# Tamerkobba/Parallel-CNN

Hardware: AMD Instinct MI355X
Metric: training images/sec (whole node) (higher is better)
Workload: dtype bf16; 1 GPU; model=LeNet-5 28x28x1 (conv6x5x5 -> trainable-pool4x4 -> fc216x10), global_batch=64, per_gpu_batch=64, input=28x28x1, parallelism=dp1, dist_backend=none, pool=trainable, loss=residual, backend=hip, hipgraph=False, overlap_comm=False

## Files before the change

csrc/bindings.cpp:

```cpp

#include <torch/extension.h>

#include <cmath>

#include "lenet_dims.h"
#include "pcnn_launch.h"

namespace pcnn {
void cpu_forward(at::Tensor x, at::Tensor params, at::Tensor a1, at::Tensor a2,
                 at::Tensor y, int64_t pool_mode, int64_t loss_mode);
double cpu_backward(at::Tensor x, at::Tensor params, at::Tensor a1,
                    at::Tensor a2, at::Tensor y, at::Tensor labels,
                    at::Tensor dz, at::Tensor dz2, at::Tensor dz1,
                    at::Tensor grads, int64_t pool_mode, int64_t loss_mode);
void cpu_update(at::Tensor params, at::Tensor grads, double dt, double scale);
void cpu_update_momentum(at::Tensor params, at::Tensor grads, at::Tensor vel,
                         double dt, double scale, double mu, double wd,
                         bool nesterov);
void cpu_update_adam(at::Tensor params, at::Tensor grads, at::Tensor m,
                     at::Tensor sq, double dt, double scale, double beta1,
                     double beta2, double eps, double wd, int64_t t);
}

namespace {
// ... 200 lines not shown
void hip_wgrad_update_adam(at::Tensor x, at::Tensor a1, at::Tensor a2,
                           at::Tensor dz, at::Tensor dz2, at::Tensor dz1,
                           at::Tensor grads, at::Tensor params, at::Tensor m,
                           at::Tensor sq, double dt, double scale,
                           double beta1, double beta2, double eps, double wd,
                           int64_t t, at::Tensor ticket, int64_t B,
                           int64_t chunk_imgs, int64_t roles,
                           int64_t stream) {
  wgrad_update_impl(
      x, a1, a2, dz, dz2, dz1, grads, params,
      adam_opt(m, sq, params, dt, scale, beta1, beta2, eps, wd, t), ticket, B,
      chunk_imgs, roles, stream, "wgrad_update_adam");
}

float* gslab_ptr(const at::Tensor& gslab, int64_t B) {
  TORCH_CHECK(gslab.is_cuda() && gslab.scalar_type() == at::kFloat &&
                  gslab.is_contiguous() &&
                  gslab.numel() >= B * pcnn::GSLAB_LD,
              "gslab must be a contiguous device fp32 [>=B, ",
              pcnn::GSLAB_LD, "] tensor");
  return gslab.data_ptr<float>();
}

int inblock_variant(int64_t variant) {
  TORCH_CHECK(variant >= -1 && variant <= 1,
              "variant must be -1 (default), 0 (cell) or 1 (pair)");
  return (int)variant;
}

void hip_fwdbwd_inblock(at::Tensor x, at::Tensor params, at::Tensor a2,
                        at::Tensor y, at::Tensor dz, at::Tensor labels,
                        at::Tensor loss_accum, at::Tensor gslab, int64_t B,
                        int64_t stream, int64_t pool_mode,
                        int64_t loss_mode, int64_t variant) {
  TORCH_CHECK(x.is_cuda() && params.is_cuda(), "expected device tensors");
  TORCH_CHECK(labels.scalar_type() == at::kInt, "labels must be int32");
  TORCH_CHECK(B >= 1 && x.numel() >= B * pcnn::IN_PIX &&
                  a2.numel() >= B * pcnn::S1_OUT &&
                  a2.scalar_type() == x.scalar_type() &&
                  y.numel() >= B * pcnn::FC_OUT &&
                  dz.numel() >= B * pcnn::FC_OUT && labels.numel() >= B,
              "buffers too small for B");
  check_hip(pcnn_launch_fwdbwd_inblock(
                x.data_ptr(), params.data_ptr<float>(), a2.data_ptr(),
                y.data_ptr<float>(), dz.data_ptr<float>(),
                labels.data_ptr<int>(),
                loss_accum.numel() ? loss_accum.data_ptr<float>() : nullptr,
                gslab_ptr(gslab, B), (int)B, act_flag(x), (int)pool_mode,
                (int)loss_mode, inblock_variant(variant), (void*)stream),
            "fwdbwd_inblock");
}

void step_inblock_impl(const at::Tensor& x, const at::Tensor& params,
                       const at::Tensor& a1, const at::Tensor& a2,
                       const at::Tensor& y, const at::Tensor& dz,
                       const at::Tensor& dz2, const at::Tensor& dz1,
                       const at::Tensor& labels, const at::Tensor& loss_accum,
                       const at::Tensor& grads, const at::Tensor& ticket,
                       const at::Tensor& gslab, const pcnn_opt& opt,
                       int64_t B, int64_t chunk_imgs, int64_t stream,
                       int64_t pool_mode, int64_t loss_mode, int64_t variant,
                       const char* what) {
  TORCH_CHECK(x.is_cuda() && params.is_cuda(), "expected device tensors");
  TORCH_CHECK(labels.scalar_type() == at::kInt, "labels must be int32");
  TORCH_CHECK(dz1.scalar_type() == x.scalar_type() &&
                  a2.scalar_type() == x.scalar_type(),
              "a2/dz1 must match the activation dtype");
  TORCH_CHECK(params.numel() == pcnn::N_PARAMS &&
                  grads.numel() == pcnn::N_PARAMS,
              "params/grads must be the flat device buckets");
  TORCH_CHECK(B >= 1 && x.numel() >= B * pcnn::IN_PIX &&
                  a2.numel() >= B * pcnn::S1_OUT &&
                  y.numel() >= B * pcnn::FC_OUT &&
                  dz.numel() >= B * pcnn::FC_OUT && labels.numel() >= B,
              "buffers too small for B");
  TORCH_CHECK(B <= pcnn_inblock_max_batch() ||
                  (a1.numel() >= B * pcnn::C1_OUT &&
                   dz1.numel() >= B * pcnn::C1_OUT &&
                   dz2.numel() >= B * pcnn::S1_OUT),
              "a1/dz1/dz2 too small for the large-batch path");
  check_hip(pcnn_launch_step_inblock(
                x.data_ptr(), params.data_ptr<float>(), a1.data_ptr(),
                a2.data_ptr(), y.data_ptr<float>(), dz.data_ptr<float>(),
                dz2.data_ptr<float>(), dz1.data_ptr(), labels.data_ptr<int>(),
                loss_accum.data_ptr<float>(), grads.data_ptr<float>(),
                ticket_ptr(ticket), gslab_ptr(gslab, B), &opt, (int)B,
                act_flag(x), (int)pool_mode, (int)loss_mode, (int)chunk_imgs,
                inblock_variant(variant), (void*)stream),
            what);
}

void hip_step_inblock(at::Tensor x, at::Tensor params, at::Tensor a1,
                      at::Tensor a2, at::Tensor y, at::Tensor dz,
                      at::Tensor dz2, at::Tensor dz1, at::Tensor labels,
                      at::Tensor loss_accum, at::Tensor grads,
                      at::Tensor ticket, at::Tensor gslab, double step,
                      int64_t B, int64_t chunk_imgs, int64_t stream,
                      int64_t pool_mode, int64_t loss_mode,
                      int64_t variant) {
  step_inblock_impl(x, params, a1, a2, y, dz, dz2, dz1, labels, loss_accum,
                    grads, ticket, gslab, plain_opt(step), B, chunk_imgs,
                    stream, pool_mode, loss_mode, variant, "step_inblock");
}

void hip_step_inblock_momentum(at::Tensor x, at::Tensor params,
                               at::Tensor vel, at::Tensor a1, at::Tensor a2,
                               at::Tensor y, at::Tensor dz, at::Tensor dz2,
                               at::Tensor dz1, at::Tensor labels,
                               at::Tensor loss_accum, at::Tensor grads,
                               at::Tensor ticket, at::Tensor gslab, double dt,
                               double scale, double mu, double wd,
                               bool nesterov, int64_t B, int64_t chunk_imgs,
                               int64_t stream, int64_t pool_mode,
                               int64_t loss_mode, int64_t variant) {
  step_inblock_impl(x, params, a1, a2, y, dz, dz2, dz1, labels, loss_accum,
                    grads, ticket, gslab,
                    momentum_opt(vel, params, dt, scale, mu, wd, nesterov), B,
                    chunk_imgs, stream, pool_mode, loss_mode, variant,
                    "step_inblock_momentum");
}

void hip_step_inblock_adam(at::Tensor x, at::Tensor params, at::Tensor m,
                           at::Tensor sq, at::Tensor a1, at::Tensor a2,
                           at::Tensor y, at::Tensor dz, at::Tensor dz2,
                           at::Tensor dz1, at::Tensor labels,
                           at::Tensor loss_accum, at::Tensor grads,
                           at::Tensor ticket, at::Tensor gslab, double dt,
                           double scale, double beta1, double beta2,
                           double eps, double wd, int64_t t, int64_t B,
                           int64_t chunk_imgs, int64_t stream,
                           int64_t pool_mode, int64_t loss_mode,
                           int64_t variant) {
  step_inblock_impl(
      x, params, a1, a2, y, dz, dz2, dz1, labels, loss_accum, grads, ticket,
      gslab, adam_opt(m, sq, params, dt, scale, beta1, beta2, eps, wd, t), B,
      chunk_imgs, stream, pool_mode, loss_mode, variant, "step_inblock_adam");
}

void reduce_update_impl(const at::Tensor& gslab, const at::Tensor& a2,
                        const at::Tensor& dz, const at::Tensor& params,
                        const pcnn_opt& opt, int64_t B, int64_t stream,
                        const char* what) {
  TORCH_CHECK(params.is_cuda() && params.numel() == pcnn::N_PARAMS,
              "params must be the flat device bucket");
  TORCH_CHECK(B >= 1 && a2.is_cuda() && a2.numel() >= B * pcnn::S1_OUT &&
                  dz.is_cuda() && dz.scalar_type() == at::kFloat &&
                  dz.numel() >= B * pcnn::FC_OUT,
              "buffers too small for B");
  check_hip(pcnn_launch_reduce_update(gslab_ptr(gslab, B), a2.data_ptr(),
                                      dz.data_ptr<float>(),
                                      params.data_ptr<float>(), &opt, (int)B,
                                      act_flag(a2), (void*)stream),
            what);
}

void hip_reduce_update_momentum(at::Tensor gslab, at::Tensor a2,
                                at::Tensor dz, at::Tensor params,
                                at::Tensor vel, double dt, double scale,
                                double mu, double wd, bool nesterov,
                                int64_t B, int64_t stream) {
  reduce_update_impl(gslab, a2, dz, params,
                     momentum_opt(vel, params, dt, scale, mu, wd, nesterov),
                     B, stream, "reduce_update_momentum");
}

void hip_reduce_update_adam(at::Tensor gslab, at::Tensor a2, at::Tensor dz,
                            at::Tensor params, at::Tensor m, at::Tensor sq,
                            double dt, double scale, double beta1,
                            double beta2, double eps, double wd, int64_t t,
                            int64_t B, int64_t stream) {
  reduce_update_impl(
      gslab, a2, dz, params,
      adam_opt(m, sq, params, dt, scale, beta1, beta2, eps, wd, t), B, stream,
      "reduce_update_adam");
}

void hip_train_steps(at::Tensor x_pool, at::Tensor labels_pool,
                     at::Tensor params, at::Tensor grads, at::Tensor a1,
                     at::Tensor a2, at::Tensor y, at::Tensor dz,
                     at::Tensor dz2, at::Tensor dz1, at::Tensor loss_accum,
                     int64_t B, int64_t steps, int64_t chunk_imgs,
                     double step_scale, int64_t stream, int64_t pool_mode,
                     int64_t loss_mode, int64_t wgrad_fuse,
                     int64_t step_mode, at::Tensor ticket,
                     at::Tensor gslab, at::Tensor vel, double dt,
                     double scale, double mu, double wd, bool nesterov,
                     int64_t variant, at::Tensor sq, double beta2, double eps,
                     int64_t t0) {
  const int var = inblock_variant(variant);
  const bool adam = sq.numel() != 0;
  TORCH_CHECK(!adam || t0 >= 0, "t0 is the number of updates applied so far");
  pcnn_opt opt =
      adam ? adam_opt(vel, sq, params, dt, scale, mu, beta2, eps, wd, t0 + 1)
      : vel.numel() ? momentum_opt(vel, params, dt, scale, mu, wd, nesterov)
                    : plain_opt(step_scale);
  TORCH_CHECK(step_mode == 3 || step_mode == 2 || step_mode == 4,
              "step_mode must be 3, 2 or 4");
  TORCH_CHECK(step_mode == 3 || !wgrad_fuse,
              "the two-launch steps exclude wgrad_fuse");
  int* tk = step_mode != 3 ? ticket_ptr(ticket) : nullptr;
  float* slab = step_mode == 4 ? gslab_ptr(gslab, B) : nullptr;
  const int wroles = wgrad_fuse ? 4 : (pool_mode == 1 ? 5 : 7);
  TORCH_CHECK(x_pool.is_cuda() && x_pool.dim() == 2, "x_pool [P*B, 784]");
  TORCH_CHECK(labels_pool.scalar_type() == at::kInt, "labels must be int32");
  const int64_t pool_rows = x_pool.size(0);
  TORCH_CHECK(pool_rows % B == 0, "pool rows must be a multiple of B");
  const int64_t P = pool_rows / B;
  const int f = act_flag(x_pool);
  const size_t esz = f ? 2 : 4;
  const char* xp = (const char*)x_pool.data_ptr();
  const int* lp = labels_pool.data_ptr<int>();
  float* pp = params.data_ptr<float>();
  float* gp = grads.data_ptr<float>();
  void* s = (void*)stream;
  for (int64_t st = 0; st < steps; ++st) {
    const int64_t i = st % P;
    const void* xb = xp + (size_t)i * B * pcnn::IN_PIX * esz;
    const int* lb = lp + i * B;
    if (adam && st > 0)
      opt = adam_opt(vel, sq, params, dt, scale, mu, beta2, eps, wd,
                     t0 + st + 1);
    if (step_mode == 4) {
      check_hip(pcnn_launch_step_inblock(
                    xb, pp, a1.data_ptr(), a2.data_ptr(), y.data_ptr<float>(),
                    dz.data_ptr<float>(), dz2.data_ptr<float>(),
                    dz1.data_ptr(), lb, loss_accum.data_ptr<float>(), gp, tk,
                    slab, &opt, (int)B, f, (int)pool_mode, (int)loss_mode,
                    (int)chunk_imgs, var, s),
                "train_steps/step_inblock");
      continue;
    }
    check_hip(pcnn_launch_fwdbwd(xb, pp, a1.data_ptr(), a2.data_ptr(),
                                 y.data_ptr<float>(), dz.data_ptr<float>(),
                                 dz2.data_ptr<float>(), dz1.data_ptr(), lb,
                                 loss_accum.data_ptr<float>(), nullptr,
                                 (int)B, f, 0, (int)pool_mode, (int)loss_mode,
                                 gp, (int)wgrad_fuse, s),
              "train_steps/fwdbwd");
    if (step_mode == 2) {
      check_hip(pcnn_launch_wgrad_update(
                    xb, a1.data_ptr(), a2.data_ptr(), dz.data_ptr<float>(),
                    dz2.data_ptr<float>(), dz1.data_ptr(), gp, pp, &opt, tk,
                    (int)B, f, (int)chunk_imgs, wroles, s),
                "train_steps/wgrad_update");
      continue;
    }
    check_hip(pcnn_launch_wgrad(xb, a1.data_ptr(), a2.data_ptr(),
                                dz.data_ptr<float>(), dz2.data_ptr<float>(),
                                dz1.data_ptr(), gp, (int)B, f,
                                (int)chunk_imgs, wroles, s),
              "train_steps/wgrad");
    check_hip(pcnn_launch_update(pp, gp, &opt, s), "train_steps/update");
  }
}

void deep_im2col(at::Tensor x, at::Tensor cols, int64_t B, int64_t H,
                 int64_t W, int64_t Cin, int64_t K, int64_t P, int64_t KcP,
                 int64_t stream) {
  check_hip(pcnn_deep_im2col(x.data_ptr(), cols.data_ptr(), (int)B, (int)H,
                             (int)W, (int)Cin, (int)K, (int)P, (int)KcP,
                             act_flag(x), (void*)stream),
            "deep_im2col");
}

void deep_gemm(at::Tensor A, at::Tensor Bsrc, at::Tensor bias, at::Tensor C,
               int64_t M, int64_t K, int64_t N, int64_t ldA, int64_t ldC,
               int64_t b_kxn, int64_t epilogue, int64_t stream,
               at::Tensor Bpre, at::Tensor imx, int64_t XH, int64_t XW,
               int64_t XC, int64_t XK, int64_t XP, at::Tensor epi,
               at::Tensor pw, at::Tensor pout, int64_t PK, at::Tensor c32) {
  check_hip(pcnn_deep_gemm(
                A.data_ptr(), Bsrc.data_ptr<float>(),
                Bpre.numel() ? Bpre.data_ptr() : nullptr,
                bias.numel() ? bias.data_ptr<float>() : nullptr,
                C.data_ptr(), M, (int)K, (int)N, (int)ldA, (int)ldC,
                (int)b_kxn, (int)epilogue,
                imx.numel() ? imx.data_ptr() : nullptr, (int)XH, (int)XW,
                (int)XC, (int)XK, (int)XP,
                epi.numel() ? epi.data_ptr() : nullptr,
                pw.numel() ? pw.data_ptr<float>() : nullptr,
                pout.numel() ? pout.data_ptr() : nullptr, (int)PK,
                c32.numel() ? c32.data_ptr<float>() : nullptr,
                (long long)c32.numel(), act_flag(A), (void*)stream),
            "deep_gemm");
}

void deep_cast_wt(at::Tensor W, at::Tensor out, at::Tensor outT, int64_t R,
                  int64_t C, int64_t stream) {
  check_hip(pcnn_deep_cast_wt(W.data_ptr<float>(), out.data_ptr(),
                              outT.data_ptr(), (int)R, (int)C,
                              (void*)stream),
            "deep_cast_wt");
}

struct CastDesc {
  int R[8], C[8], K[8], Cin[8];
  long long w_off[8], bf_off[8], bfT_off[8], rot_off[8], p8_off[8];
  pcnn_cast_desc d;

  CastDesc(const char* what, const std::vector<int64_t>& Rv,
           const std::vector<int64_t>& Cv, const std::vector<int64_t>& Kv,
           const std::vector<int64_t>& Cinv, const std::vector<int64_t>& w,
           const std::vector<int64_t>& bf, const std::vector<int64_t>& bfT,
           const std::vector<int64_t>& rot, const std::vector<int64_t>& p8) {
    const size_t n = Rv.size();
    TORCH_CHECK(n >= 1 && n <= 8, what, ": 1..8 stages");
// ... 237 lines not shown
  check_hip(pcnn_deep_fc_fwd(
                flat.data_ptr(), fw.data_ptr<float>(), fb.data_ptr<float>(),
                labels.data_ptr<int>(),
                y.numel() ? y.data_ptr<float>() : nullptr,
                dz.numel() ? dz.data_ptr<float>() : nullptr,
                loss_accum.numel() ? loss_accum.data_ptr<float>() : nullptr,
                correct_accum.numel() ? correct_accum.data_ptr<int>()
                                      : nullptr,
                (int)B, (int)FCIN, (int)NCLS, (int)mode,
                dflat.numel() ? dflat.data_ptr() : nullptr, act_flag(flat),
                (void*)stream),
            "deep_fc_fwd");
}

void deep_fc_bwd(at::Tensor dz, at::Tensor flat, at::Tensor fw,
                 at::Tensor dflat, int64_t B, int64_t FCIN, int64_t NCLS,
                 int64_t stream) {
  check_hip(pcnn_deep_fc_bwd(dz.data_ptr<float>(), flat.data_ptr(),
                             fw.data_ptr<float>(), dflat.data_ptr(), (int)B,
                             (int)FCIN, (int)NCLS, act_flag(flat),
                             (void*)stream),
            "deep_fc_bwd");
}

void deep_fc_wgrad(at::Tensor dz, at::Tensor flat, at::Tensor gfw,
                   at::Tensor gfb, int64_t B, int64_t FCIN, int64_t NCLS,
                   int64_t FS, int64_t stream) {
  check_hip(pcnn_deep_fc_wgrad(dz.data_ptr<float>(), flat.data_ptr(),
                               gfw.data_ptr<float>(), gfb.data_ptr<float>(),
                               (int)B, (int)FCIN, (int)NCLS, (int)FS,
                               act_flag(flat), (void*)stream),
            "deep_fc_wgrad");
}

void deep_update(at::Tensor params, at::Tensor grads, double step,
                 int64_t stream) {
  const pcnn_opt opt = plain_opt(step);
  check_hip(pcnn_deep_update(params.data_ptr<float>(),
                             grads.data_ptr<float>(), params.numel(), &opt,
                             (void*)stream),
            "deep_update");
}

void deep_update_momentum(at::Tensor params, at::Tensor grads,
                          at::Tensor vel, double dt, double scale, double mu,
                          double wd, bool nesterov, int64_t stream) {
  TORCH_CHECK(grads.numel() == params.numel(), "grads/params size mismatch");
  const pcnn_opt opt = momentum_opt(vel, params, dt, scale, mu, wd, nesterov);
  check_hip(pcnn_deep_update(params.data_ptr<float>(),
                             grads.data_ptr<float>(), params.numel(), &opt,
                             (void*)stream),
            "deep_update_momentum");
}

void deep_update_adam(at::Tensor params, at::Tensor grads, at::Tensor m,
                      at::Tensor sq, double dt, double scale, double beta1,
                      double beta2, double eps, double wd, int64_t t,
                      int64_t stream) {
  TORCH_CHECK(grads.numel() == params.numel(), "grads/params size mismatch");
  const pcnn_opt opt =
      adam_opt(m, sq, params, dt, scale, beta1, beta2, eps, wd, t);
  check_hip(pcnn_deep_update(params.data_ptr<float>(),
                             grads.data_ptr<float>(), params.numel(), &opt,
                             (void*)stream),
            "deep_update_adam");
}

void deep_mfma_selftest(at::Tensor A, at::Tensor Bm, at::Tensor D,
                        int64_t stream) {
  check_hip(pcnn_deep_mfma_selftest(A.data_ptr<float>(),
                                    Bm.data_ptr<float>(),
                                    D.data_ptr<float>(), (void*)stream),
            "deep_mfma_selftest");
}


}

PYBIND11_MODULE(TORCH_EXTENSION_NAME, m) {
  m.doc() = "parallel_cnn_amd native ops (CPU reference + gfx950 HIP kernels)";
  m.def("cpu_forward", &pcnn::cpu_forward, py::arg("x"), py::arg("params"),
        py::arg("a1"), py::arg("a2"), py::arg("y"), py::arg("pool_mode") = 0,
        py::arg("loss_mode") = 0);
  m.def("cpu_backward", &pcnn::cpu_backward, py::arg("x"), py::arg("params"),
        py::arg("a1"), py::arg("a2"), py::arg("y"), py::arg("labels"),
        py::arg("dz"), py::arg("dz2"), py::arg("dz1"), py::arg("grads"),
        py::arg("pool_mode") = 0, py::arg("loss_mode") = 0);
  m.def("cpu_update", &pcnn::cpu_update);
  m.def("cpu_update_momentum", &pcnn::cpu_update_momentum, py::arg("params"),
        py::arg("grads"), py::arg("vel"), py::arg("dt"), py::arg("scale"),
        py::arg("mu"), py::arg("wd"), py::arg("nesterov"));
  m.def("cpu_update_adam", &pcnn::cpu_update_adam, py::arg("params"),
        py::arg("grads"), py::arg("m"), py::arg("sq"), py::arg("dt"),
        py::arg("scale"), py::arg("beta1"), py::arg("beta2"), py::arg("eps"),
        py::arg("wd"), py::arg("t"));
  m.def("hip_fwdbwd", &hip_fwdbwd, py::arg("x"), py::arg("params"),
        py::arg("a1"), py::arg("a2"), py::arg("y"), py::arg("dz"),
        py::arg("dz2"), py::arg("dz1"), py::arg("labels"),
        py::arg("loss_accum"), py::arg("correct_accum"), py::arg("B"),
        py::arg("mode"), py::arg("stream"), py::arg("pool_mode") = 0,
        py::arg("loss_mode") = 0, py::arg("grads") = at::empty({0}),
        py::arg("wgrad_fuse") = 0);
  m.def("hip_wgrad", &hip_wgrad);
  m.def("hip_wgrad_roles", &hip_wgrad_roles);
  m.def("hip_update", &hip_update);
  m.def("hip_train_steps", &hip_train_steps, py::arg("x_pool"),
        py::arg("labels_pool"), py::arg("params"), py::arg("grads"),
        py::arg("a1"), py::arg("a2"), py::arg("y"), py::arg("dz"),
        py::arg("dz2"), py::arg("dz1"), py::arg("loss_accum"), py::arg("B"),
        py::arg("steps"), py::arg("chunk_imgs"), py::arg("step_scale"),
        py::arg("stream"), py::arg("pool_mode") = 0,
        py::arg("loss_mode") = 0, py::arg("wgrad_fuse") = 0,
        py::arg("step_mode") = 3, py::arg("ticket") = at::empty({0}),
        py::arg("gslab") = at::empty({0}), py::arg("vel") = at::empty({0}),
        py::arg("dt") = 0.0, py::arg("scale") = 1.0, py::arg("mu") = 0.0,
        py::arg("wd") = 0.0, py::arg("nesterov") = false,
        py::arg("variant") = -1, py::arg("sq") = at::empty({0}),
        py::arg("beta2") = 0.999, py::arg("eps") = 1e-8, py::arg("t0") = 0);
  m.def("hip_update_adam", &hip_update_adam, py::arg("params"),
        py::arg("grads"), py::arg("m"), py::arg("sq"), py::arg("dt"),
        py::arg("scale"), py::arg("beta1"), py::arg("beta2"), py::arg("eps"),
        py::arg("wd"), py::arg("t"), py::arg("stream"));
  m.def("hip_wgrad_update_adam", &hip_wgrad_update_adam, py::arg("x"),
        py::arg("a1"), py::arg("a2"), py::arg("dz"), py::arg("dz2"),
        py::arg("dz1"), py::arg("grads"), py::arg("params"), py::arg("m"),
        py::arg("sq"), py::arg("dt"), py::arg("scale"), py::arg("beta1"),
        py::arg("beta2"), py::arg("eps"), py::arg("wd"), py::arg("t"),
        py::arg("ticket"), py::arg("B"), py::arg("chunk_imgs"),
        py::arg("roles"), py::arg("stream"));
  m.def("hip_reduce_update_adam", &hip_reduce_update_adam, py::arg("gslab"),
        py::arg("a2"), py::arg("dz"), py::arg("params"), py::arg("m"),
        py::arg("sq"), py::arg("dt"), py::arg("scale"), py::arg("beta1"),
        py::arg("beta2"), py::arg("eps"), py::arg("wd"), py::arg("t"),
        py::arg("B"), py::arg("stream"));
  m.def("hip_step_inblock_adam", &hip_step_inblock_adam, py::arg("x"),
        py::arg("params"), py::arg("m"), py::arg("sq"), py::arg("a1"),
        py::arg("a2"), py::arg("y"), py::arg("dz"), py::arg("dz2"),
        py::arg("dz1"), py::arg("labels"), py::arg("loss_accum"),
        py::arg("grads"), py::arg("ticket"), py::arg("gslab"), py::arg("dt"),
        py::arg("scale"), py::arg("beta1"), py::arg("beta2"), py::arg("eps"),
        py::arg("wd"), py::arg("t"), py::arg("B"), py::arg("chunk_imgs"),
        py::arg("stream"), py::arg("pool_mode") = 0,
        py::arg("loss_mode") = 0, py::arg("variant") = -1);
  m.def("hip_update_momentum", &hip_update_momentum, py::arg("params"),
        py::arg("grads"), py::arg("vel"), py::arg("dt"), py::arg("scale"),
        py::arg("mu"), py::arg("wd"), py::arg("nesterov"),
        py::arg("stream"));
  m.def("hip_wgrad_update_momentum", &hip_wgrad_update_momentum,
        py::arg("x"), py::arg("a1"), py::arg("a2"), py::arg("dz"),
        py::arg("dz2"), py::arg("dz1"), py::arg("grads"), py::arg("params"),
        py::arg("vel"), py::arg("dt"), py::arg("scale"), py::arg("mu"),
        py::arg("wd"), py::arg("nesterov"), py::arg("ticket"), py::arg("B"),
        py::arg("chunk_imgs"), py::arg("roles"), py::arg("stream"));
  m.def("hip_reduce_update_momentum", &hip_reduce_update_momentum,
        py::arg("gslab"), py::arg("a2"), py::arg("dz"), py::arg("params"),
        py::arg("vel"), py::arg("dt"), py::arg("scale"), py::arg("mu"),
        py::arg("wd"), py::arg("nesterov"), py::arg("B"), py::arg("stream"));
  m.def("hip_step_inblock_momentum", &hip_step_inblock_momentum,
        py::arg("x"), py::arg("params"), py::arg("vel"), py::arg("a1"),
        py::arg("a2"), py::arg("y"), py::arg("dz"), py::arg("dz2"),
        py::arg("dz1"), py::arg("labels"), py::arg("loss_accum"),
        py::arg("grads"), py::arg("ticket"), py::arg("gslab"), py::arg("dt"),
        py::arg("scale"), py::arg("mu"), py::arg("wd"), py::arg("nesterov"),
        py::arg("B"), py::arg("chunk_imgs"), py::arg("stream"),
        py::arg("pool_mode") = 0, py::arg("loss_mode") = 0,
        py::arg("variant") = -1);
  m.def("hip_fwdbwd_inblock", &hip_fwdbwd_inblock, py::arg("x"),
        py::arg("params"), py::arg("a2"), py::arg("y"), py::arg("dz"),
        py::arg("labels"), py::arg("loss_accum"), py::arg("gslab"),
        py::arg("B"), py::arg("stream"), py::arg("pool_mode") = 0,
        py::arg("loss_mode") = 0, py::arg("variant") = -1);
  m.def("hip_step_inblock", &hip_step_inblock, py::arg("x"),
        py::arg("params"), py::arg("a1"), py::arg("a2"), py::arg("y"),
        py::arg("dz"), py::arg("dz2"), py::arg("dz1"), py::arg("labels"),
        py::arg("loss_accum"), py::arg("grads"), py::arg("ticket"),
        py::arg("gslab"), py::arg("step"), py::arg("B"),
        py::arg("chunk_imgs"), py::arg("stream"), py::arg("pool_mode") = 0,
        py::arg("loss_mode") = 0, py::arg("variant") = -1);
  m.def("hip_wgrad_update", &hip_wgrad_update, py::arg("x"), py::arg("a1"),
        py::arg("a2"), py::arg("dz"), py::arg("dz2"), py::arg("dz1"),
        py::arg("grads"), py::arg("params"), py::arg("step"),
        py::arg("ticket"), py::arg("B"), py::arg("chunk_imgs"),
        py::arg("roles"), py::arg("stream"));
  m.def("deep_im2col", &deep_im2col);
  m.def("deep_gemm", &deep_gemm, py::arg("A"), py::arg("Bsrc"),
        py::arg("bias"), py::arg("C"), py::arg("M"), py::arg("K"),
        py::arg("N"), py::arg("ldA"), py::arg("ldC"), py::arg("b_kxn"),
        py::arg("epilogue"), py::arg("stream"),
        py::arg("Bpre") = at::empty({0}),
        py::arg("imx") = at::empty({0}), py::arg("XH") = 0,
        py::arg("XW") = 0, py::arg("XC") = 0, py::arg("XK") = 0,
        py::arg("XP") = 0, py::arg("epi") = at::empty({0}),
        py::arg("pw") = at::empty({0}), py::arg("pout") = at::empty({0}),
        py::arg("PK") = 0, py::arg("c32") = at::empty({0}));
  m.def("deep_cast_wt", &deep_cast_wt);
  m.def("deep_cast_all", &deep_cast_all);
  m.def("deep_pad_channels", &deep_pad_channels);
  m.def("deep_update_cast", &deep_update_cast);
  m.def("deep_wgrad_multi", &deep_wgrad_multi);
  m.def("deep_remap_dw8", &deep_remap_dw8);
  m.def("deep_wgrad_gemm", &deep_wgrad_gemm, py::arg("cols"),
        py::arg("dpre"), py::arg("dW"), py::arg("M"), py::arg("KcP"),
        py::arg("N"), py::arg("MS"), py::arg("stream"),
        py::arg("imx") = at::empty({0}), py::arg("XH") = 0,
        py::arg("XW") = 0, py::arg("XC") = 0, py::arg("XK") = 0,
        py::arg("XP") = 0, py::arg("part") = at::empty({0}),
        py::arg("db") = at::empty({0}));
  m.def("deep_colsum", &deep_colsum);
  m.def("deep_col2im_sigbwd", &deep_col2im_sigbwd);
  m.def("deep_pool_fwd", &deep_pool_fwd);
  m.def("deep_pool_bwd", &deep_pool_bwd);
  m.def("deep_pool_wgrad", &deep_pool_wgrad);
  m.def("deep_pool_wbwd", &deep_pool_wbwd);
  m.def("deep_fc_fwd", &deep_fc_fwd, py::arg("flat"), py::arg("fw"),
        py::arg("fb"), py::arg("labels"), py::arg("y"), py::arg("dz"),
        py::arg("loss_accum"), py::arg("correct_accum"), py::arg("B"),
        py::arg("FCIN"), py::arg("NCLS"), py::arg("mode"),
        py::arg("stream"), py::arg("dflat") = at::empty({0}));
  m.def("deep_fc_bwd", &deep_fc_bwd);
  m.def("deep_fc_wgrad", &deep_fc_wgrad);
  m.def("deep_update", &deep_update);
  m.def("deep_update_momentum", &deep_update_momentum);
  m.def("deep_update_cast_momentum", &deep_update_cast_momentum);
  m.def("deep_update_adam", &deep_update_adam);
  m.def("deep_update_cast_adam", &deep_update_cast_adam);
  m.def("deep_mfma_selftest", &deep_mfma_selftest);
  m.attr("N_PARAMS") = pcnn::N_PARAMS;
  m.attr("GSLAB_LD") = pcnn::GSLAB_LD;
  m.attr("INBLOCK_MAX_BATCH") = pcnn_inblock_max_batch();
  m.attr("INBLOCK_DEFAULT_VARIANT") = pcnn_inblock_default_variant();
  m.attr("OFF_C1W") = pcnn::OFF_C1W;
  m.attr("OFF_C1B") = pcnn::OFF_C1B;
  m.attr("OFF_S1W") = pcnn::OFF_S1W;
  m.attr("OFF_S1B") = pcnn::OFF_S1B;
  m.attr("OFF_FW") = pcnn::OFF_FW;
  m.attr("OFF_FB") = pcnn::OFF_FB;
  m.attr("REF_DT") = pcnn::REF_DT;
  m.attr("REF_THRESHOLD") = pcnn::REF_THRESHOLD;
  m.attr("HAS_HIP_KERNELS") = true;
}
```

csrc/hip/lenet_kernels.hip:

```cpp

#include <hip/hip_bf16.h>
#include <hip/hip_fp16.h>
#include <hip/hip_runtime.h>

#include "../lenet_dims.h"
#include "../pcnn_launch.h"
#include "act_dispatch.h"

namespace pcnn {

using bf16 = __hip_bfloat16;
using fp16 = __half;

#include "sgd_update.h"

__device__ __forceinline__ float sigmoidf_dev(float v) {
  return 1.0f / (1.0f + __expf(-v));
}

template <typename T>
__device__ __forceinline__ float ldf(const T* p) {
  return (float)*p;
}
template <typename T>
// ... 928 lines not shown
        __hip_atomic_store(&grads[OFF_FW + q], grads[OFF_FW + q] + acc,
                           __ATOMIC_RELAXED, __HIP_MEMORY_SCOPE_AGENT);
      else if (FS == 1)
        grads[OFF_FW + q] += acc;
      else
        unsafeAtomicAdd(&grads[OFF_FW + q], acc);
    } else if (q < FC_WSZ + FC_OUT) {
      const int k = q - FC_WSZ;
      float acc = 0.f;
#pragma unroll 8
      for (int b = b_lo; b < b_hi; ++b) acc += dzg[(size_t)b * FC_OUT + k];
      if (FS == 1 && WT)
        __hip_atomic_store(&grads[OFF_FB + k], grads[OFF_FB + k] + acc,
                           __ATOMIC_RELAXED, __HIP_MEMORY_SCOPE_AGENT);
      else if (FS == 1)
        grads[OFF_FB + k] += acc;
      else
        unsafeAtomicAdd(&grads[OFF_FB + k], acc);
    }
  }
}

template <typename act_t>
__global__ __launch_bounds__(256) void k_wgrad(
    const act_t* __restrict__ x, const act_t* __restrict__ a1g,
    const act_t* __restrict__ a2g, const float* __restrict__ dzg,
    const float* __restrict__ dz2g, const act_t* __restrict__ dz1g,
    float* __restrict__ grads, int B, int GC, int GS, int FS, int roles) {
  wgrad_body<act_t, false>(x, a1g, a2g, dzg, dz2g, dz1g, grads, B, GC, GS,
                           FS, roles);
}

__device__ __forceinline__ bool arrive_is_last(int* __restrict__ ticket) {
  __shared__ int s_last;
  asm volatile("s_waitcnt vmcnt(0)" ::: "memory");
  __syncthreads();
  if (threadIdx.x == 0) {
    const int t = __hip_atomic_fetch_add(ticket, 1, __ATOMIC_RELAXED,
                                         __HIP_MEMORY_SCOPE_AGENT);
    const int last = (t == (int)gridDim.x - 1);
    if (last) {
      __builtin_amdgcn_fence(__ATOMIC_ACQUIRE, "agent");
      asm volatile("s_waitcnt vmcnt(0)" ::: "memory");
    }
    s_last = last;
  }
  __syncthreads();
  return s_last != 0;
}

template <int OPT, typename Args>
__device__ __forceinline__ void update_tail(float* __restrict__ params,
                                            float* __restrict__ grads,
                                            float* __restrict__ vel,
                                            float* __restrict__ sq,
                                            float step, const Args& o) {
  constexpr int NV = N_PARAMS / 4;
  for (int i4 = threadIdx.x; i4 < NV; i4 += 256)
    sgd_apply4<OPT>(params, grads, vel, sq, i4 * 4, step, o);
  const int u = NV * 4 + threadIdx.x;
  if (u < N_PARAMS) sgd_apply1<OPT>(params, grads, vel, sq, u, step, o);
}

template <typename act_t, int OPT, typename Args>
__device__ __forceinline__ void wgrad_update_body(
    const act_t* __restrict__ x, const act_t* __restrict__ a1g,
    const act_t* __restrict__ a2g, const float* __restrict__ dzg,
    const float* __restrict__ dz2g, const act_t* __restrict__ dz1g,
    float* __restrict__ grads, int B, int GC, int GS, int FS, int roles,
    float* __restrict__ params, float step, float* __restrict__ vel,
    float* __restrict__ sq, const Args& o, int* __restrict__ ticket) {
  wgrad_body<act_t, true>(x, a1g, a2g, dzg, dz2g, dz1g, grads, B, GC, GS,
                          FS, roles);
  if (!arrive_is_last(ticket)) return;
  update_tail<OPT>(params, grads, vel, sq, step, o);
  if (threadIdx.x == 0)
    __hip_atomic_store(ticket, 0, __ATOMIC_RELAXED, __HIP_MEMORY_SCOPE_AGENT);
}

template <typename act_t>
__global__ __launch_bounds__(256) void k_wgrad_update_mom(
    const act_t* __restrict__ x, const act_t* __restrict__ a1g,
    const act_t* __restrict__ a2g, const float* __restrict__ dzg,
    const float* __restrict__ dz2g, const act_t* __restrict__ dz1g,
    float* __restrict__ grads, int B, int GC, int GS, int FS, int roles,
    float* __restrict__ params, float* __restrict__ vel, MomArgs o,
    int* __restrict__ ticket) {
  wgrad_update_body<act_t, OPT_MOM>(x, a1g, a2g, dzg, dz2g, dz1g, grads, B,
                                    GC, GS, FS, roles, params, 0.f, vel,
                                    nullptr, o, ticket);
}

template <typename act_t>
__global__ __launch_bounds__(256) void k_wgrad_update_adam(
    const act_t* __restrict__ x, const act_t* __restrict__ a1g,
    const act_t* __restrict__ a2g, const float* __restrict__ dzg,
    const float* __restrict__ dz2g, const act_t* __restrict__ dz1g,
    float* __restrict__ grads, int B, int GC, int GS, int FS, int roles,
    float* __restrict__ params, float* __restrict__ vel,
    float* __restrict__ sq, AdamArgs o, int* __restrict__ ticket) {
  wgrad_update_body<act_t, OPT_ADAM>(x, a1g, a2g, dzg, dz2g, dz1g, grads, B,
                                     GC, GS, FS, roles, params, 0.f, vel, sq,
                                     o, ticket);
}

template <typename act_t>
__global__ __launch_bounds__(256) void k_wgrad_update(
    const act_t* __restrict__ x, const act_t* __restrict__ a1g,
    const act_t* __restrict__ a2g, const float* __restrict__ dzg,
    const float* __restrict__ dz2g, const act_t* __restrict__ dz1g,
    float* __restrict__ grads, int B, int GC, int GS, int FS, int roles,
    float* __restrict__ params, float step, int* __restrict__ ticket) {
  wgrad_update_body<act_t, OPT_PLAIN>(x, a1g, a2g, dzg, dz2g, dz1g, grads, B,
                                      GC, GS, FS, roles, params, step,
                                      nullptr, nullptr, MomArgs{}, ticket);
}

template <int OPT, typename Args>
__device__ __forceinline__ void update_body(float* __restrict__ params,
                                            float* __restrict__ grads,
                                            float* __restrict__ vel,
                                            float* __restrict__ sq,
                                            float step, const Args& o) {
  const int i4 = blockIdx.x * 256 + threadIdx.x;
  const int i = i4 * 4;
  if (i + 3 < N_PARAMS) {
    sgd_apply4<OPT>(params, grads, vel, sq, i, step, o);
  } else if (i < N_PARAMS) {
    for (int u = i; u < N_PARAMS; ++u)
      sgd_apply1<OPT>(params, grads, vel, sq, u, step, o);
  }
}

__global__ __launch_bounds__(256) void k_update(float* __restrict__ params,
                                                float* __restrict__ grads,
                                                float step) {
  update_body<OPT_PLAIN>(params, grads, nullptr, nullptr, step, MomArgs{});
}

__global__ __launch_bounds__(256) void k_update_mom(
    float* __restrict__ params, float* __restrict__ grads,
    float* __restrict__ vel, MomArgs o) {
  update_body<OPT_MOM>(params, grads, vel, nullptr, 0.f, o);
}

__global__ __launch_bounds__(256) void k_update_adam(
    float* __restrict__ params, float* __restrict__ grads,
    float* __restrict__ vel, float* __restrict__ sq, AdamArgs o) {
  update_body<OPT_ADAM>(params, grads, vel, sq, 0.f, o);
}


constexpr int RU_LANES = 4;
constexpr int RU_DEPTH = 8;
constexpr int RU_PARAMS_PER_BLOCK = 256 / RU_LANES;
constexpr int RU_BLOCKS =
    (N_PARAMS + RU_PARAMS_PER_BLOCK - 1) / RU_PARAMS_PER_BLOCK;
constexpr int INBLOCK_MAX_B = 256;
constexpr int INBLOCK_DEFAULT_VARIANT = 1;

template <typename act_t, int OPT, typename Args>
__device__ __forceinline__ void reduce_update_body(
    const float* __restrict__ gslab, const act_t* __restrict__ a2g,
    const float* __restrict__ dzg, float* __restrict__ params, float step,
    int B, float* __restrict__ vel, float* __restrict__ sq, const Args& o) {
  const int p = blockIdx.x * RU_PARAMS_PER_BLOCK + (threadIdx.x >> 2);
  const int sub = threadIdx.x & (RU_LANES - 1);
  const int pc = p < N_PARAMS ? p : N_PARAMS - 1;
  constexpr int STEP_B = RU_LANES * RU_DEPTH;
  float acc = 0.f;
  if (pc < OFF_FW) {
    for (int b0 = sub; b0 < B; b0 += STEP_B) {
      float v[RU_DEPTH];
#pragma unroll
      for (int u = 0; u < RU_DEPTH; ++u) {
        const int b = b0 + u * RU_LANES;
        const int bc = b < B ? b : B - 1;
        v[u] = gslab[(size_t)bc * GSLAB_LD + pc];
        if (b >= B) v[u] = 0.f;
      }
#pragma unroll
      for (int u = 0; u < RU_DEPTH; ++u) acc += v[u];
    }
  } else if (pc < OFF_FB) {
    const int q = pc - OFF_FW;
    const int k = q / FC_IN;
    const int m = q - k * FC_IN;
    for (int b0 = sub; b0 < B; b0 += STEP_B) {
      float d[RU_DEPTH], a[RU_DEPTH];
#pragma unroll
      for (int u = 0; u < RU_DEPTH; ++u) {
        const int b = b0 + u * RU_LANES;
        const int bc = b < B ? b : B - 1;
        d[u] = dzg[(size_t)bc * FC_OUT + k];
        a[u] = ldf(a2g + (size_t)bc * FC_IN + m);
        if (b >= B) d[u] = 0.f;
      }
#pragma unroll
      for (int u = 0; u < RU_DEPTH; ++u) acc += d[u] * a[u];
    }
  } else {
    const int k = pc - OFF_FB;
    for (int b0 = sub; b0 < B; b0 += STEP_B) {
      float d[RU_DEPTH];
#pragma unroll
      for (int u = 0; u < RU_DEPTH; ++u) {
        const int b = b0 + u * RU_LANES;
        const int bc = b < B ? b : B - 1;
        d[u] = dzg[(size_t)bc * FC_OUT + k];
        if (b >= B) d[u] = 0.f;
      }
#pragma unroll
      for (int u = 0; u < RU_DEPTH; ++u) acc += d[u];
    }
  }
  acc += __shfl_xor(acc, 1, RU_LANES);
  acc += __shfl_xor(acc, 2, RU_LANES);
  if (sub == 0 && p < N_PARAMS) {
    if constexpr (OPT == OPT_ADAM) {
      float m = vel[p], s = sq[p];
      params[p] = adam_apply(params[p], acc, m, s, o);
      vel[p] = m;
      sq[p] = s;
    } else if constexpr (OPT == OPT_MOM) {
      float v = vel[p];
      params[p] = mom_apply(params[p], acc, v, o);
      vel[p] = v;
    } else {
      params[p] += step * acc;
    }
  }
}

template <typename act_t>
__global__ __launch_bounds__(256) void k_reduce_update(
    const float* __restrict__ gslab, const act_t* __restrict__ a2g,
    const float* __restrict__ dzg, float* __restrict__ params, float step,
    int B) {
  reduce_update_body<act_t, OPT_PLAIN>(gslab, a2g, dzg, params, step, B,
                                       nullptr, nullptr, MomArgs{});
}

template <typename act_t>
__global__ __launch_bounds__(256) void k_reduce_update_mom(
    const float* __restrict__ gslab, const act_t* __restrict__ a2g,
    const float* __restrict__ dzg, float* __restrict__ params,
    float* __restrict__ vel, MomArgs o, int B) {
  reduce_update_body<act_t, OPT_MOM>(gslab, a2g, dzg, params, 0.f, B, vel,
                                     nullptr, o);
}

template <typename act_t>
__global__ __launch_bounds__(256) void k_reduce_update_adam(
    const float* __restrict__ gslab, const act_t* __restrict__ a2g,
    const float* __restrict__ dzg, float* __restrict__ params,
    float* __restrict__ vel, float* __restrict__ sq, AdamArgs o, int B) {
  reduce_update_body<act_t, OPT_ADAM>(gslab, a2g, dzg, params, 0.f, B, vel,
                                      sq, o);
}

}


using namespace pcnn;

namespace {
template <int MODE>
int launch_fwdbwd_mode(const void* x, const float* params, void* a1, void* a2,
                       float* y, float* dz, float* dz2, void* dz1,
                       const int* labels, float* loss_accum, int* correct,
                       int B, int act, int pool_mode, int loss_mode,
                       float* grads, int wgrad_fuse, hipStream_t stream) {
  dim3 grid(B), block(256);
  PCNN_DISPATCH(act, hipLaunchKernelGGL(
                         (k_fwdbwd<act_t, MODE>), grid, block, 0, stream,
                         (const act_t*)x, params, (act_t*)a1, (act_t*)a2, y,
                         dz, dz2, (act_t*)dz1, labels, loss_accum, correct, B,
                         pool_mode, loss_mode, grads, wgrad_fuse));
  return (int)hipGetLastError();
}

int launch_wgrad_any(const void* x, const void* a1, const void* a2,
                     const float* dz, const float* dz2, const void* dz1,
                     float* grads, int B, int act, int chunk_imgs, int roles,
                     float* params, const pcnn_opt* opt, int* ticket,
                     hipStream_t s) {
  int GC = chunk_imgs > 0 ? chunk_imgs : (int)(4.0f * __builtin_cbrtf((float)B) + 0.5f);
  if (GC < 2) GC = 2;
  if (GC > 256) GC = 256;
  if (roles == 4) GC = 0;
  int GS = (B * S1_OUT + 256 * 5 - 1) / (256 * 5);
  if (GS < 2) GS = 2;
  if (GS > 96) GS = 96;
  if (roles == 4) GS = 0;
  int FS = B / 64;
  if (FS < 1) FS = 1;
  if (FS > 32) FS = 32;
  dim3 grid(C1_CH * GC + GS + FS * FC_BLOCKS), block(256);
  const int sel = ticket == nullptr ? OPT_PLAIN : opt_select(opt);
  if (sel < 0) return (int)hipErrorInvalidValue;
  PCNN_DISPATCH(act, {
    const act_t *xs = (const act_t*)x, *a1s = (const act_t*)a1,
                *a2s = (const act_t*)a2, *dz1s = (const act_t*)dz1;
    if (ticket == nullptr)
      hipLaunchKernelGGL((k_wgrad<act_t>), grid, block, 0, s, xs, a1s, a2s,
                         dz, dz2, dz1s, grads, B, GC, GS, FS, roles);
    else if (sel == OPT_ADAM)
      hipLaunchKernelGGL((k_wgrad_update_adam<act_t>), grid, block, 0, s, xs,
                         a1s, a2s, dz, dz2, dz1s, grads, B, GC, GS, FS, roles,
                         params, opt->vel, opt->sq, adam_args(opt), ticket);
    else if (sel == OPT_MOM)
      hipLaunchKernelGGL((k_wgrad_update_mom<act_t>), grid, block, 0, s, xs,
                         a1s, a2s, dz, dz2, dz1s, grads, B, GC, GS, FS, roles,
                         params, opt->vel, mom_args(opt), ticket);
    else
      hipLaunchKernelGGL((k_wgrad_update<act_t>), grid, block, 0, s, xs, a1s,
                         a2s, dz, dz2, dz1s, grads, B, GC, GS, FS, roles,
                         params, opt->step, ticket);
  });
  return (int)hipGetLastError();
}
}

extern "C" {

int pcnn_launch_fwdbwd(const void* x, const float* params, void* a1, void* a2,
                       float* y, float* dz, float* dz2, void* dz1,
                       const int* labels, float* loss_accum, int* correct,
                       int B, int act, int mode, int pool_mode, int loss_mode,
                       float* grads, int wgrad_fuse, void* stream) {
  hipStream_t s = (hipStream_t)stream;
  switch (mode) {
    case MODE_TRAIN:
      return launch_fwdbwd_mode<MODE_TRAIN>(x, params, a1, a2, y, dz, dz2,
                                            dz1, labels, loss_accum, correct,
                                            B, act, pool_mode, loss_mode,
                                            grads, wgrad_fuse, s);
    case MODE_EVAL:
      return launch_fwdbwd_mode<MODE_EVAL>(x, params, a1, a2, y, dz, dz2, dz1,
                                           labels, loss_accum, correct, B,
                                           act, pool_mode, loss_mode, grads,
                                           wgrad_fuse, s);
    default:
      return launch_fwdbwd_mode<MODE_INFER>(x, params, a1, a2, y, dz, dz2,
                                            dz1, labels, loss_accum, correct,
                                            B, act, pool_mode, loss_mode,
                                            grads, wgrad_fuse, s);
  }
}

int pcnn_launch_wgrad(const void* x, const void* a1, const void* a2,
                      const float* dz, const float* dz2, const void* dz1,
                      float* grads, int B, int act, int chunk_imgs, int roles,
                      void* stream) {
  return launch_wgrad_any(x, a1, a2, dz, dz2, dz1, grads, B, act, chunk_imgs,
                          roles, nullptr, nullptr, nullptr,
                          (hipStream_t)stream);
}

int pcnn_launch_update(float* params, float* grads, const pcnn_opt* opt,
                       void* stream) {
  if (opt == nullptr) return (int)hipErrorInvalidValue;
  dim3 grid((N_PARAMS / 4 + 255) / 256), block(256);
  const int sel = opt_select(opt);
  if (sel < 0) return (int)hipErrorInvalidValue;
  if (sel == OPT_ADAM)
    hipLaunchKernelGGL(k_update_adam, grid, block, 0, (hipStream_t)stream,
                       params, grads, opt->vel, opt->sq, adam_args(opt));
  else if (sel == OPT_MOM)
    hipLaunchKernelGGL(k_update_mom, grid, block, 0, (hipStream_t)stream,
                       params, grads, opt->vel, mom_args(opt));
  else
    hipLaunchKernelGGL(k_update, grid, block, 0, (hipStream_t)stream, params,
                       grads, opt->step);
  return (int)hipGetLastError();
}

int pcnn_launch_wgrad_update(const void* x, const void* a1, const void* a2,
                             const float* dz, const float* dz2,
                             const void* dz1, float* grads, float* params,
                             const pcnn_opt* opt, int* ticket, int B, int act,
                             int chunk_imgs, int roles, void* stream) {
// ... 111 lines not shown
```

Before: 6.372 million images/sec.

## Software-pipeline reduce-update loads and unify branchless gradient accumulation paths

```diff
diff --git a/csrc/bindings.cpp b/csrc/bindings.cpp
--- a/csrc/bindings.cpp
+++ b/csrc/bindings.cpp
@@ -376,6 +376,13 @@
                                       params.data_ptr<float>(), &opt, (int)B,
                                       act_flag(a2), (void*)stream),
             what);
+}
+
+void hip_reduce_update(at::Tensor gslab, at::Tensor a2, at::Tensor dz,
+                       at::Tensor params, double step, int64_t B,
+                       int64_t stream) {
+  reduce_update_impl(gslab, a2, dz, params, plain_opt(step), B, stream,
+                     "reduce_update");
 }
 
 void hip_reduce_update_momentum(at::Tensor gslab, at::Tensor a2,
@@ -919,6 +926,9 @@
         py::arg("vel"), py::arg("dt"), py::arg("scale"), py::arg("mu"),
         py::arg("wd"), py::arg("nesterov"), py::arg("ticket"), py::arg("B"),
         py::arg("chunk_imgs"), py::arg("roles"), py::arg("stream"));
+  m.def("hip_reduce_update", &hip_reduce_update, py::arg("gslab"),
+        py::arg("a2"), py::arg("dz"), py::arg("params"), py::arg("step"),
+        py::arg("B"), py::arg("stream"));
   m.def("hip_reduce_update_momentum", &hip_reduce_update_momentum,
         py::arg("gslab"), py::arg("a2"), py::arg("dz"), py::arg("params"),
         py::arg("vel"), py::arg("dt"), py::arg("scale"), py::arg("mu"),
diff --git a/csrc/hip/lenet_kernels.hip b/csrc/hip/lenet_kernels.hip
--- a/csrc/hip/lenet_kernels.hip
+++ b/csrc/hip/lenet_kernels.hip
@@ -1104,82 +1104,121 @@
 
 
 constexpr int RU_LANES = 4;
-constexpr int RU_DEPTH = 8;
+constexpr int RU_DEPTH_SMALL = 8;
+constexpr int RU_DEPTH = 16;
 constexpr int RU_PARAMS_PER_BLOCK = 256 / RU_LANES;
 constexpr int RU_BLOCKS =
     (N_PARAMS + RU_PARAMS_PER_BLOCK - 1) / RU_PARAMS_PER_BLOCK;
 constexpr int INBLOCK_MAX_B = 256;
 constexpr int INBLOCK_DEFAULT_VARIANT = 1;
 
+__device__ __forceinline__ void ru_fetch_args(const MomArgs& o) {
+  asm volatile("" ::"s"(o.scale), "s"(o.dt), "s"(o.mu), "s"(o.wd),
+               "s"(o.nesterov));
+}
+__device__ __forceinline__ void ru_fetch_args(const AdamArgs& o) {
+  asm volatile("" ::"s"(o.scale), "s"(o.dt), "s"(o.beta1), "s"(o.beta2),
+               "s"(o.eps), "s"(o.wd), "s"(o.c1), "s"(o.c2), "s"(o.omb1),
+               "s"(o.omb2));
+}
+
+template <int DEPTH, typename act_t>
+__device__ __forceinline__ void ru_load(float (&d)[DEPTH], act_t (&a)[DEPTH],
+                                        const float* __restrict__ dcol,
+                                        int dld,
+                                        const act_t* __restrict__ acol,
+                                        int b0, int B) {
+#pragma unroll
+  for (int u = 0; u < DEPTH; ++u) {
+    const int b = b0 + u * RU_LANES;
+    const int bc = b < B ? b : B - 1;
+    d[u] = dcol[(size_t)bc * dld];
+    a[u] = acol[(size_t)bc * FC_IN];
+  }
+}
+template <int DEPTH, typename act_t>
+__device__ __forceinline__ float ru_add(float acc, const float (&d)[DEPTH],
+                                        const act_t (&a)[DEPTH], bool fcw,
+                                        int b0, int B) {
+#pragma unroll
+  for (int u = 0; u < DEPTH; ++u)
+    acc = __builtin_fmaf(b0 + u * RU_LANES < B ? d[u] : 0.f,
+                         fcw ? (float)a[u] : 1.0f, acc);
+  return acc;
+}
+
+template <int DEPTH, typename act_t>
+__device__ __forceinline__ float ru_sum(const float* __restrict__ dcol,
+                                        int dld,
+                                        const act_t* __restrict__ acol,
+                                        bool fcw, int sub, int B) {
+  constexpr int STEP_B = RU_LANES * DEPTH;
+  float d[DEPTH];
+  act_t a[DEPTH];
+  ru_load<DEPTH>(d, a, dcol, dld, acol, sub, B);
+  __builtin_amdgcn_sched_barrier(0);
+  float acc = 0.f;
+  int base = 0;
+  for (; base + STEP_B < B; base += STEP_B) {
+    float dn[DEPTH];
+    act_t an[DEPTH];
+    ru_load<DEPTH>(dn, an, dcol, dld, acol, base + STEP_B + sub, B);
+    __builtin_amdgcn_sched_barrier(0);
+    acc = ru_add<DEPTH>(acc, d, a, fcw, base + sub, B);
+#pragma unroll
+    for (int u = 0; u < DEPTH; ++u) {
+      d[u] = dn[u];
+      a[u] = an[u];
+    }
+  }
+  return ru_add<DEPTH>(acc, d, a, fcw, base + sub, B);
+}
+
 template <typename act_t, int OPT, typename Args>
 __device__ __forceinline__ void reduce_update_body(
     const float* __restrict__ gslab, const act_t* __restrict__ a2g,
     const float* __restrict__ dzg, float* __restrict__ params, float step,
     int B, float* __restrict__ vel, float* __restrict__ sq, const Args& o) {
+  asm volatile("" ::"s"(gslab), "s"(a2g), "s"(dzg), "s"(params), "s"(B));
+  if constexpr (OPT == OPT_PLAIN) asm volatile("" ::"s"(step));
+  if constexpr (OPT != OPT_PLAIN) {
+    asm volatile("" ::"s"(vel));
+    ru_fetch_args(o);
+  }
+  if constexpr (OPT == OPT_ADAM) asm volatile("" ::"s"(sq));
   const int p = blockIdx.x * RU_PARAMS_PER_BLOCK + (threadIdx.x >> 2);
   const int sub = threadIdx.x & (RU_LANES - 1);
   const int pc = p < N_PARAMS ? p : N_PARAMS - 1;
-  constexpr int STEP_B = RU_LANES * RU_DEPTH;
-  float acc = 0.f;
-  if (pc < OFF_FW) {
-    for (int b0 = sub; b0 < B; b0 += STEP_B) {
-      float v[RU_DEPTH];
-#pragma unroll
-      for (int u = 0; u < RU_DEPTH; ++u) {
-        const int b = b0 + u * RU_LANES;
-        const int bc = b < B ? b : B - 1;
-        v[u] = gslab[(size_t)bc * GSLAB_LD + pc];
-        if (b >= B) v[u] = 0.f;
-      }
-#pragma unroll
-      for (int u = 0; u < RU_DEPTH; ++u) acc += v[u];
-    }
-  } else if (pc < OFF_FB) {
-    const int q = pc - OFF_FW;
-    const int k = q / FC_IN;
-    const int m = q - k * FC_IN;
-    for (int b0 = sub; b0 < B; b0 += STEP_B) {
-      float d[RU_DEPTH], a[RU_DEPTH];
-#pragma unroll
-      for (int u = 0; u < RU_DEPTH; ++u) {
-        const int b = b0 + u * RU_LANES;
-        const int bc = b < B ? b : B - 1;
-        d[u] = dzg[(size_t)bc * FC_OUT + k];
-        a[u] = ldf(a2g + (size_t)bc * FC_IN + m);
-        if (b >= B) d[u] = 0.f;
-      }
-#pragma unroll
-      for (int u = 0; u < RU_DEPTH; ++u) acc += d[u] * a[u];
-    }
-  } else {
-    const int k = pc - OFF_FB;
-    for (int b0 = sub; b0 < B; b0 += STEP_B) {
-      float d[RU_DEPTH];
-#pragma unroll
-      for (int u = 0; u < RU_DEPTH; ++u) {
-        const int b = b0 + u * RU_LANES;
-        const int bc = b < B ? b : B - 1;
-        d[u] = dzg[(size_t)bc * FC_OUT + k];
-        if (b >= B) d[u] = 0.f;
-      }
-#pragma unroll
-      for (int u = 0; u < RU_DEPTH; ++u) acc += d[u];
-    }
-  }
+  float pv = params[pc];
+  float mv = 0.f, sv = 0.f;
+  if constexpr (OPT != OPT_PLAIN) mv = vel[pc];
+  if constexpr (OPT == OPT_ADAM) sv = sq[pc];
+  const bool slab = pc < OFF_FW;
+  const bool fcw = !slab && pc < OFF_FB;
+  const int q = fcw ? pc - OFF_FW : 0;
+  const int k = fcw ? q / FC_IN : (slab ? 0 : pc - OFF_FB);
+  const int m = q - (fcw ? k : 0) * FC_IN;
+  const float* dcol = slab ? gslab + pc : dzg + k;
+  const int dld = slab ? GSLAB_LD : FC_OUT;
+  const act_t* acol = a2g + m;
+  float acc = B <= RU_LANES * RU_DEPTH_SMALL
+                  ? ru_sum<RU_DEPTH_SMALL>(dcol, dld, acol, fcw, sub, B)
+                  : ru_sum<RU_DEPTH>(dcol, dld, acol, fcw, sub, B);
+  asm volatile("" : "+v"(pv));
+  if constexpr (OPT != OPT_PLAIN) asm volatile("" : "+v"(mv));
+  if constexpr (OPT == OPT_ADAM) asm volatile("" : "+v"(sv));
   acc += __shfl_xor(acc, 1, RU_LANES);
   acc += __shfl_xor(acc, 2, RU_LANES);
   if (sub == 0 && p < N_PARAMS) {
     if constexpr (OPT == OPT_ADAM) {
-      float m = vel[p], s = sq[p];
-      params[p] = adam_apply(params[p], acc, m, s, o);
-      vel[p] = m;
-      sq[p] = s;
+      params[p] = adam_apply(pv, acc, mv, sv, o);
+      vel[p] = mv;
+      sq[p] = sv;
     } else if constexpr (OPT == OPT_MOM) {
-      float v = vel[p];
-      params[p] = mom_apply(params[p], acc, v, o);
-      vel[p] = v;
+      params[p] = mom_apply(pv, acc, mv, o);
+      vel[p] = mv;
     } else {
-      params[p] += step * acc;
+      params[p] = __builtin_fmaf(step, acc, pv);
     }
   }
 }
```

Result: faster. 6.724 million images/sec (median of 6 runs) (+5.5%).
